# ooshyun/Speech-Enhancement-Pytorch

Measured on AMD Instinct MI355X. Metric: audio-sec/sec training, DCCRN 16kHz 2s bs32, higher is better.
Workload: dtype bf16; 1 GPU; DCCRN (kernel_num 16-32-64-128-256-256, complex LSTM 128, mask E) train step, 16 kHz 2-s clips, SI-SNR, Adam 3e-4, clip 5; per_gpu_batch=32, global_batch=32, samples_per_clip=32000, parallelism=dp1, launch=eager, inputs=resident in HBM

## Files before the change

### include/sehip.h

```cpp
#ifndef SEHIP_H
#define SEHIP_H
#include <stdint.h>

#ifdef __cplusplus
extern "C" {
#endif

const char* sehip_last_error(void);
const char* sehip_last_kernel(void);
int sehip_version(void);
int sehip_check_device(int device);

void* sehip_event_create(void);
int sehip_event_destroy(void* event);
int sehip_stream_depend(void* to_stream, void* from_stream, void* event);
int sehip_event_record(void* event, void* stream);
int sehip_stream_wait_event(void* stream, void* event);
void* sehip_stream_create(int priority_class);
int sehip_stream_destroy(void* stream);

int sehip_stft_frames(int n_samples, int win_len, int hop);
int sehip_stft_fwd(const float* wav , const float* window , int B, int N, int win_len, int hop,
                   int fft_len, float* spec , void* enc_in_bf16 , void* stream);
int sehip_istft_fwd(const float* spec, const float* mask , const float* window,
                    const float* inv_coff , int B, int T, int win_len, int hop, int fft_len, int length,
                    int masking_mode , float* frames_ws , float* wav ,
                    void* stream);
int sehip_istft_bwd(const float* dwav, const float* wav, const float* spec, const float* mask, const float* window,
                    const float* inv_coff, int B, int T, int win_len, int hop, int fft_len, int length,
                    int masking_mode, void* dmask_bf16 , void* stream);

int sehip_stft_custom_frames(int n_samples, int n_fft, int hop, int center);
int sehip_stft_custom_fwd(const float* wav, int rows, int n_samples, int n_fft, int hop, int win_length, int center,
                          float* spec, void* stream);
int sehip_istft_custom_fwd(const float* spec, int rows, int n_frames, int n_fft, int hop, int win_length, int center,
                           int length, float* frames_ws, float* wav, void* stream);

int sehip_wav_row_stats(const float* raw, const long* row_off, int rows, float* stats, void* stream);
int sehip_wav_collate(const float* raw, const long* row_off, const int* out_row, const long* out_start, const int* out_valid,
                      const float* stats, int mode, float eps, int seg, int out_rows, float* out, void* stream);

int sehip_sisnr_fwd(const float* est, const float* ref, int rows, int n, float* rowstat, float* loss, void* stream);
int sehip_sisdr_metric(const float* reference, const float* estimation, int rows, int n, float* ratios, float* out, void* stream);
int sehip_sisnr_bwd(const float* est, const float* ref, const float* rowstat, const float* upstream ,
                    int rows, int n, float* dest, void* stream);

int sehip_sisnr_pit_fwd(const float* est, const float* ref, int B, int S, int C, int n, float* rowstat, float* pairloss,
                        int* perm, float* loss, void* stream);
int sehip_sisnr_pit_bwd(const float* est, const float* ref, const float* rowstat, const int* perm, const float* upstream ,
                        int B, int S, int C, int n, float* dest, void* stream);

int sehip_psa_loss_fwd(const float* enh, const float* tgt, const float* mix, long ncomplex, double* acc, float* loss, void* stream);
int sehip_psa_loss_bwd(const float* enh, const float* tgt, const float* mix, long ncomplex, const float* upstream, float* denh, void* stream);
int sehip_pointwise_loss_fwd(const float* x, const float* y, long n, int mode, double* acc_scratch, float* loss, void* stream);
int sehip_pointwise_loss_bwd(const float* x, const float* y, long n, int mode, const float* upstream, float* dx, void* stream);

int sehip_grad_sumsq(const float* grads, long n, double* sumsq_out, void* stream);
int sehip_opt_step(float* params, float* grads, float* m, float* v, long n, const double* sumsq, float max_norm,
                   float lr, float beta1, float beta2, float eps, int step, const int* step_dev ,
                   float weight_decay, int mode, float grad_scale, void* stream);
// ... 297 lines not shown
```

### speech-enhancement-pytorch_amd/sehip/_lib.py

```python
import ctypes as C
import os

import torch

_HERE = os.path.dirname(os.path.abspath(__file__))
LIB_PATH = os.environ.get("SEHIP_LIB") or os.path.join(_HERE, "libsehip.so")


class SehipError(RuntimeError):
    pass


_lib = None

P = C.c_void_p
I = C.c_int
L = C.c_long
F = C.c_float
U = C.c_uint

_PROTOS = {
    "sehip_version": [],
    "sehip_check_device": [I],
    "sehip_set_deterministic": [I],
# ... 12 lines not shown
    "sehip_comm_unique_id": [P],
    "sehip_comm_init": [P, I, I, P],
    "sehip_allreduce_f32": [P, P, L, P],
    "sehip_allreduce_i32_max": [P, P, L, P],
    "sehip_comm_info": [P, P, P, P],
    "sehip_comm_destroy": [P],
    "sehip_wav_row_stats": [P, P, I, P, P],
    "sehip_wav_collate": [P, P, P, P, P, P, I, F, I, I, P, P],
    "sehip_sisnr_fwd": [P, P, I, I, P, P, P],
    "sehip_sisdr_metric": [P, P, I, I, P, P, P],
    "sehip_sisnr_bwd": [P, P, P, P, I, I, P, P],
    "sehip_sisnr_pit_fwd": [P, P, I, I, I, I, P, P, P, P, P],
    "sehip_sisnr_pit_bwd": [P, P, P, P, P, I, I, I, I, P, P],
    "sehip_psa_loss_fwd": [P, P, P, L, P, P, P],
    "sehip_psa_loss_bwd": [P, P, P, L, P, P, P],
    "sehip_pointwise_loss_fwd": [P, P, L, I, P, P, P],
    "sehip_pointwise_loss_bwd": [P, P, L, I, P, P, P],
    "sehip_grad_sumsq": [P, L, P, P],
    "sehip_opt_step": [P, P, P, P, L, P, F, F, F, F, F, I, P, F, I, F, P],
    "sehip_opt_step_g": [P, P, P, P, L, P, F, F, F, F, F, I, P, F, I, F, P, P],
    "sehip_opt_step_m": [P, P, P, P, L, P, F, F, F, F, F, I, P, F, I, F, P, P, I, P, P, P, P],
    "sehip_opt_begin_g": [P, I, P, P, I, P, P],
    "sehip_counter_add": [P, I, P],
    "sehip_zero_regions": [P, L, P, L, P, L, P, L, P],
    "sehip_gemm_takes_gln_stats": [P],
    "sehip_init": [],
    "sehip_grad_metric": [P, P, I, L, P, P, P, P],
    "sehip_opt_begin": [P, I, P, P, I, P],
    "sehip_grad_sumsq_acc": [P, L, P, P],
    "sehip_grad_metric_acc": [P, P, I, L, P, P, P, P],
    "sehip_cbn_scratch_floats": [L, I],
    "sehip_stft_fwd": [P, P, I, I, I, I, I, P, P, P],
    "sehip_istft_fwd": [P, P, P, P, I, I, I, I, I, I, I, P, P, P],
    "sehip_istft_bwd": [P, P, P, P, P, P, I, I, I, I, I, I, I, P, P],
    "sehip_gemm": [P, P],
    "sehip_gemm_pair": [P, P, P],
    "sehip_wgrad": [P, P],
    "sehip_wgrad_pair": [P, P, P],
    "sehip_bnr_rows": [P, P],
    "sehip_cbn_bwd_finalize_n": [P, I, P, P, P, P, L, I, P, P, P, P, P, P, P, P],
    "sehip_wgrad_group_bytes": [I],
    "sehip_wgrad_group_prepare": [P, I, P, P],
    "sehip_wgrad_group": [P, I, I, P],
    "sehip_wgrad_dense_group_bytes": [I],
    "sehip_wgrad_dense_group_prepare": [P, I, P, L, P],
    "sehip_wgrad_dense_group": [P, I, P, P, P],
    "sehip_gemm_desc_size": [],
    "sehip_conv_small_takes": [P, P],
    "sehip_pack_bf16": [P, P, L, P, P],
    "sehip_pack_f32": [P, P, L, P, P],
    "sehip_pack_head": [P, P, L, P, P, L, P, P, L, P],
    "sehip_unpack_grad": [P, P, L, P, P],
    "sehip_unpack_grad_sums": [P, P, L, P, P, I, P, P, P, P, P],
    "sehip_unpack_grad_sums_perm": [P, P, P, L, P, P, I, P, P, P, P, P],
    "sehip_unpack_grad1": [P, P, L, P, P],
    "sehip_unpack_grad1_sums": [P, P, L, P, P, I, P, P, P, P, P],
    "sehip_unpack_grad_list_sums": [P, P, P, L, P, P, I, P, P, P],
    "sehip_unpack_grad_list": [P, P, P, L, P, P],
    "sehip_pack_bf16_runs": [P, P, P, L, P, P],
    "sehip_pack_bf16_runs_to": [P, P, P, P, L, P, P],
    "sehip_cbn_stats": [P, L, I, P, P],
    "sehip_cbn_finalize": [P, P, P, P, P, P, P, P, P, P, P, P, L, I, F, F, I, P, P],
    "sehip_cbn_finalize_n": [P, I, P, P, P, P, P, P, P, P, P, P, P, L, I, F, F, I, P, P],
    "sehip_cbn_apply": [P, P, P, L, I, P, P],
    "sehip_cbn_finalize_apply_n": [P, P, I, P, P, P, P, P, P, P, P, P, P, P, L, I, F, F, I, P, P, P, P],
    "sehip_cbn_bwd_reduce": [P, P, P, P, P, L, I, I, I, I, P, P],
# ... 155 lines not shown
```

### speech-enhancement-pytorch_amd/sehip/csrc/stft.hip

```cpp
#include "common.h"

#include "fft512.h"
#include "mask.h"

__global__ __launch_bounds__(256) void stft_fwd_kernel(const float* __restrict__ wav, const float* __restrict__ window,
                                                       int B, int N, int T, int win, int hop,
                                                       float2* __restrict__ spec, unsigned* __restrict__ enc_in) {
    const int lane = threadIdx.x & 63;
    const int frame = blockIdx.x * 4 + (threadIdx.x >> 6);
    if (frame >= B * T) return;
    const int b = frame / T, t = frame - b * T;
    FftTw tw;
    fft_twiddles<-1>(tw, lane);
    float re[8], im[8];
    const int pad = win - hop;
    const float* x = wav + (size_t)b * N;
#pragma unroll
    for (int r = 0; r < 8; ++r) {
        const int n = lane + 64 * r;
        const int s = t * hop + n - pad;
        float v = 0.f;
        if (n < win && s >= 0 && s < N) v = x[s] * window[n];
        re[r] = v; im[r] = 0.f;
    }
    fft512_wave<-1>(re, im, tw, lane);
    __shared__ float2 srow[4][264 + 33];
    __shared__ unsigned senc[4][256];
    const int w = threadIdx.x >> 6;
    const int k0 = 8 * brev6(lane);
    constexpr int brev3[8] = {0, 4, 2, 6, 1, 5, 3, 7};
    if (k0 <= 256) {
#pragma unroll
        for (int j = 0; j < 8; ++j) {
            const int k = k0 + brev3[j];
            if (k <= 256) {
                srow[w][k + (k >> 3)] = make_float2(re[j], im[j]);
                if (k >= 1) senc[w][k - 1] = pack_bf2(re[j], im[j]);
            }
        }
    }
    __builtin_amdgcn_fence(__ATOMIC_RELEASE, "wavefront");
    __builtin_amdgcn_wave_barrier();
    __builtin_amdgcn_fence(__ATOMIC_ACQUIRE, "wavefront");
    float2* so = spec + (size_t)frame * NBIN;
    unsigned* eo = enc_in + (size_t)frame * 256;
#pragma unroll
    for (int j = 0; j < 4; ++j) {
        const int k = lane + 64 * j;
        so[k] = srow[w][k + (k >> 3)];
    }
    if (lane == 0) so[256] = srow[w][256 + 32];
    *reinterpret_cast<uint4*>(eo + 4 * lane) = *reinterpret_cast<const uint4*>(&senc[w][4 * lane]);
}

__global__ __launch_bounds__(256) void istft_frames_kernel(const float2* __restrict__ spec, const float2* __restrict__ mask,
                                                           const float* __restrict__ window, int nframes, int win, int mode,
                                                           float* __restrict__ frames) {
    const int lane = threadIdx.x & 63;
    const int frame = blockIdx.x * 4 + (threadIdx.x >> 6);
    if (frame >= nframes) return;
    FftTw tw;
    fft_twiddles<1>(tw, lane);
    float re[8], im[8];
    const float2* sp = spec + (size_t)frame * NBIN;
    const float2* mk = mask + (size_t)frame * 256;
#pragma unroll
    for (int r = 0; r < 8; ++r) {
        const int k = lane + 64 * r;
        float er = 0.f, ei = 0.f;
        if (k >= 1 && k <= 256) {
            const float2 z = sp[k];
            const float2 m = mk[k - 1];
            apply_mask(mode, z.x, z.y, m.x, m.y, er, ei);
        }
        re[r] = er; im[r] = ei;
    }
    fft512_wave<1>(re, im, tw, lane);
    const int n0 = 8 * brev6(lane);
    constexpr int brev3[8] = {0, 4, 2, 6, 1, 5, 3, 7};
    float u[8];
    float s1 = 0.f, s2 = 0.f;
#pragma unroll
    for (int j = 0; j < 8; ++j) {
        const int n = n0 + brev3[j];
        u[brev3[j]] = re[j];
        if (n < win) { s1 += re[j]; s2 += (n & 1) ? -re[j] : re[j]; }
    }
    s1 = wave_sum(s1);
    s2 = wave_sum(s2);
    const float c = 1.0f / (float)(FFT_N + win);
    float* fo = frames + (size_t)frame * win;
    if (n0 + 8 <= win && (win & 3) == 0) {
        float o[8];
#pragma unroll
        for (int q = 0; q < 8; ++q) {
            const int n = n0 + q;
            const float corr = c * (s1 + ((n & 1) ? -s2 : s2));
            o[q] = window[n] * (1.0f / 256.0f) * (u[q] - corr);
        }
        *reinterpret_cast<float4*>(fo + n0) = make_float4(o[0], o[1], o[2], o[3]);
        *reinterpret_cast<float4*>(fo + n0 + 4) = make_float4(o[4], o[5], o[6], o[7]);
        return;
    }
#pragma unroll
    for (int q = 0; q < 8; ++q) {
        const int n = n0 + q;
        if (n < win) {
            const float corr = c * (s1 + ((n & 1) ? -s2 : s2));
            fo[n] = window[n] * (1.0f / 256.0f) * (u[q] - corr);
        }
    }
}

__global__ __launch_bounds__(256) void istft_ola_kernel(const float* __restrict__ frames, const float* __restrict__ inv_coff,
                                                        int T, int win, int hop, int length, float* __restrict__ wav) {
    const int b = blockIdx.y;
    const int pad = win - hop;
    for (int i = blockIdx.x * 256 + threadIdx.x; i < length; i += gridDim.x * 256) {
        const int s = i + pad;
        int t_hi = s / hop;
        int t_lo = (s - win + hop) / hop;
        if (s - win + 1 <= 0) t_lo = 0;
        if (t_hi > T - 1) t_hi = T - 1;
        float acc = 0.f;
        for (int t = t_lo; t <= t_hi; ++t) acc += frames[((size_t)b * T + t) * win + (s - t * hop)];
        acc *= inv_coff[i];
        wav[(size_t)b * length + i] = fminf(1.f, fmaxf(-1.f, acc));
    }
}

__global__ __launch_bounds__(256) void istft_bwd_kernel(const float* __restrict__ dwav, const float* __restrict__ wav,
                                                        const float* __restrict__ inv_coff, const float* __restrict__ window,
                                                        const float2* __restrict__ spec, const float2* __restrict__ mask,
                                                        int B, int T, int win, int hop, int length, int mode,
                                                        unsigned* __restrict__ dmask_bf16) {
    const int lane = threadIdx.x & 63;
    const int frame = blockIdx.x * 4 + (threadIdx.x >> 6);
    if (frame >= B * T) return;
    const int b = frame / T, t = frame - b * T;
    FftTw tw;
    fft_twiddles<-1>(tw, lane);
    const int pad = win - hop;
    float re[8], im[8];
    float s1 = 0.f, s2 = 0.f;
#pragma unroll
    for (int r = 0; r < 8; ++r) {
        const int n = lane + 64 * r;
        const int i = t * hop + n - pad;
        float v = 0.f;
        if (n < win && i >= 0 && i < length) {
            const size_t o = (size_t)b * length + i;
            const float y = wav[o];
            if (y > -1.f && y < 1.f) v = dwav[o] * inv_coff[i] * window[n] * (1.0f / 256.0f);
        }
        re[r] = v; im[r] = 0.f;
        s1 += v; s2 += (n & 1) ? -v : v;
    }
    s1 = wave_sum(s1);
    s2 = wave_sum(s2);
    const float c = 1.0f / (float)(FFT_N + win);
#pragma unroll
    for (int r = 0; r < 8; ++r) {
        const int n = lane + 64 * r;
        if (n < win) re[r] -= c * (s1 + ((n & 1) ? -s2 : s2));
    }
    const float2* sp = spec + (size_t)frame * NBIN;
    const float2* mk = mask + (size_t)frame * 256;
    float2 spv[4], mkv[4];
#pragma unroll
    for (int j = 0; j < 4; ++j) { spv[j] = sp[1 + lane + 64 * j]; mkv[j] = mk[lane + 64 * j]; }
    fft512_wave<-1>(re, im, tw, lane);
    __shared__ float2 ssp[4][256 + 32], smk[4][256 + 32];
    __shared__ unsigned sdm[4][256];
    const int w = threadIdx.x >> 6;
#pragma unroll
    for (int j = 0; j < 4; ++j) {
        const int i = lane + 64 * j;
        ssp[w][i + (i >> 3)] = spv[j];
        smk[w][i + (i >> 3)] = mkv[j];
    }
    __builtin_amdgcn_fence(__ATOMIC_RELEASE, "wavefront");
    __builtin_amdgcn_wave_barrier();
    __builtin_amdgcn_fence(__ATOMIC_ACQUIRE, "wavefront");
    const int k0 = 8 * brev6(lane);
    constexpr int brev3[8] = {0, 4, 2, 6, 1, 5, 3, 7};
    if (k0 <= 256) {
#pragma unroll
        for (int j = 0; j < 8; ++j) {
            const int k = k0 + brev3[j];
            if (k < 1 || k > 256) continue;
            const float dr = re[j], di = im[j];
            const int i = k - 1;
            const float2 z = ssp[w][i + (i >> 3)];
            const float2 m = smk[w][i + (i >> 3)];
            float gmr, gmi;
            mask_grad(mode, z.x, z.y, m.x, m.y, dr, di, gmr, gmi);
            sdm[w][i] = pack_bf2(gmr, gmi);
        }
    }
    __builtin_amdgcn_fence(__ATOMIC_RELEASE, "wavefront");
    __builtin_amdgcn_wave_barrier();
    __builtin_amdgcn_fence(__ATOMIC_ACQUIRE, "wavefront");
    unsigned* dm = dmask_bf16 + (size_t)frame * 256;
    *reinterpret_cast<uint4*>(dm + 4 * lane) = *reinterpret_cast<const uint4*>(&sdm[w][4 * lane]);
}

static int check_stft_cfg(const char* who, int win, int hop, int fft) {
    SEHIP_REQUIRE(fft == FFT_N, "%s: only fft_len 512 is built (got %d)", who, fft);
    SEHIP_REQUIRE(win > 0 && win <= FFT_N && (win % 2) == 0, "%s: win_len must be even and <= 512 (got %d)", who, win);
    SEHIP_REQUIRE(hop > 0 && hop <= win, "%s: bad hop %d", who, hop);
    return 0;
}

extern "C" int sehip_stft_frames(int n_samples, int win, int hop) { return (n_samples + 2 * (win - hop) - win) / hop + 1; }

extern "C" int sehip_stft_fwd(const float* wav, const float* window, int B, int N, int win, int hop, int fft, float* spec,
                              void* enc_in_bf16, void* stream) {
    if (int e = check_stft_cfg("stft_fwd", win, hop, fft)) return e;
    SEHIP_REQUIRE(B > 0 && N > 0, "stft_fwd: empty input");
    const int T = sehip_stft_frames(N, win, hop);
    SEHIP_REQUIRE(T > 0, "stft_fwd: input shorter than one frame");
    stft_fwd_kernel<<<cdiv((long)B * T, 4), 256, 0, (hipStream_t)stream>>>(wav, window, B, N, T, win, hop, (float2*)spec,
                                                                           (unsigned*)enc_in_bf16);
    SEHIP_CHECK_LAUNCH("stft_fwd");
    return 0;
}

extern "C" int sehip_istft_fwd(const float* spec, const float* mask, const float* window, const float* inv_coff, int B,
                               int T, int win, int hop, int fft, int length, int mode, float* frames_ws, float* wav,
                               void* stream) {
    if (int e = check_stft_cfg("istft_fwd", win, hop, fft)) return e;
    SEHIP_REQUIRE(B > 0 && T > 0 && length > 0, "istft_fwd: empty input");
    SEHIP_REQUIRE(mode >= 0 && mode <= 2, "istft_fwd: masking mode must be 0(E) 1(C) 2(R)");
    SEHIP_REQUIRE(length <= (T - 1) * hop + win - (win - hop), "istft_fwd: length %d exceeds the synthesised signal", length);
    hipStream_t st = (hipStream_t)stream;
    istft_frames_kernel<<<cdiv((long)B * T, 4), 256, 0, st>>>((const float2*)spec, (const float2*)mask, window, B * T, win,
                                                             mode, frames_ws);
    dim3 grid(cdiv(length, 256 * 4), B);
    istft_ola_kernel<<<grid, 256, 0, st>>>(frames_ws, inv_coff, T, win, hop, length, wav);
    SEHIP_CHECK_LAUNCH("istft_fwd");
    return 0;
}

extern "C" int sehip_istft_bwd(const float* dwav, const float* wav, const float* spec, const float* mask,
                               const float* window, const float* inv_coff, int B, int T, int win, int hop, int fft,
                               int length, int mode, void* dmask_bf16, void* stream) {
    if (int e = check_stft_cfg("istft_bwd", win, hop, fft)) return e;
    SEHIP_REQUIRE(B > 0 && T > 0 && length > 0, "istft_bwd: empty input");
    SEHIP_REQUIRE(mode >= 0 && mode <= 2, "istft_bwd: masking mode must be 0(E) 1(C) 2(R)");
    istft_bwd_kernel<<<cdiv((long)B * T, 4), 256, 0, (hipStream_t)stream>>>(dwav, wav, inv_coff, window, (const float2*)spec,
                                                                            (const float2*)mask, B, T, win, hop, length, mode,
                                                                            (unsigned*)dmask_bf16);
    SEHIP_CHECK_LAUNCH("istft_bwd");
    return 0;
}
```

### speech-enhancement-pytorch_amd/sehip/model/dccrn.py

```python
import os
import numpy as np
import torch
from torch import nn

from .. import plan, ops
from .._lib import SehipError
from .flat import FlatModule, _Node

_STATIC_CACHE = {}


def _static_for(cfg, deterministic=False):
    switches = tuple(os.environ.get(k) for k in ("SEHIP_NO_FUSE_STATS", "SEHIP_NO_FUSE_STATS64", "SEHIP_NO_FUSE_STATS32", "SEHIP_DEC_SPLIT"))
    key = (tuple(cfg.kernel_num), cfg.rnn_layers, cfg.rnn_units, cfg.win_len, cfg.win_inc, cfg.fft_len, cfg.length, cfg.masking_mode, str(cfg.win_type), bool(cfg.use_cbn), bool(cfg.use_clstm), switches,
           bool(deterministic))
    if key not in _STATIC_CACHE:
        _STATIC_CACHE[key] = plan.DCCRNStatic(cfg, deterministic=deterministic)
    return _STATIC_CACHE[key]


class _DCCRNFunction(torch.autograd.Function):
    @staticmethod
    def forward(ctx, model, wav, anchor):
        ctx.model = model
        ctx.ws = model._run_forward(wav)
        ctx.generation = ctx.ws.generation
        return ctx.ws.wav.view(wav.shape[0], 1, -1).clone()

    @staticmethod
    def backward(ctx, grad_out):
        if ctx.generation != ctx.ws.generation or ctx.ws.closed:
            raise SehipError("DCCRN.backward: the workspace of this forward was overwritten by a later forward of the same "
                             "shape (or evicted); run backward before the next forward of that shape")
        from .._lib import stream_scope
        with stream_scope():
            ctx.model._run_backward(ctx.ws, grad_out)
        return None, None, None


class DCCRN(FlatModule):
    def __init__(self, rnn_layers=2, rnn_units=128, win_len=400, win_inc=100, fft_len=512, length=16384, win_type="hann",
                 masking_mode="E", use_clstm=True, use_cbn=True, kernel_size=5, kernel_num=[16, 32, 64, 128, 256, 256],
                 *args, **kwargs):
        super().__init__()
        self.cfg = cfg = plan.DCCRNConfig(rnn_layers=rnn_layers, rnn_units=rnn_units, win_len=win_len, win_inc=win_inc,
                                          fft_len=fft_len, length=length, win_type=win_type, masking_mode=masking_mode,
                                          use_clstm=use_clstm, use_cbn=use_cbn, kernel_size=kernel_size,
                                          kernel_num=list(kernel_num))
        self.win_len, self.win_inc, self.fft_len, self.rnn_units = win_len, win_inc, fft_len, rnn_units
        self.masking_mode, self.kernel_num = masking_mode, cfg.kernel_num
        self.static = _static_for(cfg)
        self._tables = None
        self._ws_cap = max(1, int(os.environ.get("SEHIP_WS_CACHE", "4")))
        self.grad_range_hook = None

        an, sy, win = _stft_bases(win_len, fft_len, win_type)
        self.stft = _Node()
        self.stft.register_buffer("weight", torch.from_numpy(an[:, None, :]))
        self.istft = _Node()
        self.istft.register_buffer("weight", torch.from_numpy(sy[:, None, :]))
# ... 36 lines not shown

    def set_deterministic(self, on=True):
        on = bool(on)
        if on == self.static.deterministic:
            return self
        self.static = _static_for(self.cfg, deterministic=on)
        self._tables = None
        for ws in list(self._ws.values()):
            ws.close()
        self._ws.clear()
        self._last_ws = None
        return self

    step_guard_early = True

    def step_guard(self):
        ws = getattr(self, "_last_ws", None)
        return ws.l2_sync[0:1] if ws is not None and hasattr(ws, "l2_sync") else None

    def check_health(self):
        from ..distrib import global_flag
        ws = getattr(self, "_last_ws", None)
        if ws is None:
            return global_flag(False, self._flat.device if self._flat is not None else None)
        lost = bool(ws.check_lstm_handoffs(recover=True, global_flag=global_flag))
        self._note_graph_epoch(ws)
        return lost

    def _run_forward(self, wav):
        ws = self.workspace(wav.shape[0], wav.shape[-1])
        self._last_ws = ws
        ws.generation += 1
        x = wav.reshape(wav.shape[0], wav.shape[-1]).contiguous().float()
        ws.forward(x, self._flat, self._bflat, self._nbt, training=self.training)
        return ws

    def _run_backward(self, ws, grad_out):
        if not self.training:
            raise SehipError("DCCRN.backward in eval mode (running-statistics BatchNorm) is not built")
        g = grad_out.reshape(ws.B, ws.length).contiguous().float()
        accumulating = self._grads_live and self._params[0][1].grad is not None
        hook = self.grad_range_hook if not accumulating else None
        tail = self._tail_sink if (hook is None and not accumulating) else None
        self._backward_into_flat(lambda dst: ws.backward(g, self._flat, dst, range_ready=hook, tail=tail))
        if tail is not None:
            self._tail_done = self._tail_counted = self._tail_dirty = True
        else:
            self._tail_done = False

    def forward(self, inputs, lens=None):
        if inputs.dim() == 2:
            inputs = inputs.unsqueeze(1)
        if not inputs.is_cuda:
            raise SehipError("DCCRN.forward got a CPU tensor: the HIP path needs a gfx950 GPU (no CPU fallback)")
        if torch.is_grad_enabled() and self.training:
            if self._anchor is None or self._anchor.device != inputs.device:
                self._anchor = torch.zeros(1, device=inputs.device, requires_grad=True)
            return _DCCRNFunction.apply(self, inputs, self._anchor)
        ws = self._run_forward(inputs)
        return ws.wav.view(inputs.shape[0], 1, -1).clone()

    def get_params(self, weight_decay=0.0):
        weights, biases = [], []
        for name, p in self.named_parameters():
            (biases if "bias" in name else weights).append(p)
        return [{"params": weights, "weight_decay": weight_decay}, {"params": biases, "weight_decay": 0.0}]


def _stft_bases(win_len, fft_len, win_type="hann"):
    n = np.arange(win_len, dtype=np.float64)[None, :]
    k = np.arange(fft_len // 2 + 1, dtype=np.float64)[:, None]
    ang = 2.0 * np.pi * k * n / fft_len
    basis = np.concatenate([np.cos(ang), -np.sin(ang)], axis=0)
    win = ops.window_of(win_type, win_len).astype(np.float64)
    return ((basis * win).astype(np.float32), (np.linalg.pinv(basis).T * win).astype(np.float32), win.astype(np.float32))
```

### speech-enhancement-pytorch_amd/sehip/plan.py

```python
import ctypes as C
import os
import math

import numpy as np
import torch

from . import _lib
from ._lib import call, ptr, stream, SehipError
from . import ops

BF16 = torch.bfloat16


class CSrc(C.Structure):
    _fields_ = [("ptr", C.c_void_p), ("T", C.c_int32), ("tlo", C.c_int32), ("thi", C.c_int32), ("F", C.c_int32),
                ("C", C.c_int32), ("pad_", C.c_int32)]


class CDst(C.Structure):
    _fields_ = [("ptr", C.c_void_p), ("T", C.c_int32), ("F", C.c_int32), ("C", C.c_int32), ("toff", C.c_int32),
                ("fmul", C.c_int32), ("fadd", C.c_int32), ("is_f32", C.c_int32), ("tmul", C.c_int32)]


class CGemmDesc(C.Structure):
# ... 794 lines not shown
                add(f"dz{i}", T, f, c)
        c5, h = kn[6], cfg.hid
        add("dz5l", T, 4, c5); add("P", T, 4, c5); add("dP", T, 4, c5)
        L = cfg.rnn_layers
        if not cfg.use_clstm:
            for layer in (1, 2):
                add(f"pre{layer}", T, 1, 4 * h, dtype=torch.float32)
                add(f"dpre{layer}", T, 1, 4 * h)
                add(f"h{layer}", T, 1, h, lead=1)
                add(f"gates{layer}", T, 1, 4 * h, lead=1, batch=Bp)
                add(f"c{layer}", T, 1, h, dtype=torch.float32, lead=1, batch=Bp)
            add("dxo", T, 1, h); add("dx2", T, 1, h)
        for layer in range(1, L + 1 if cfg.use_clstm else 0):
            for tag in "ri":
                add(f"pre{layer}_{tag}", T, 1, 8 * h, dtype=torch.float32)
                add(f"dpre{layer}_{tag}", T, 1, 8 * h)
            add(f"h{layer}", T, 1, h, lead=4)
            add(f"gates{layer}", T, 1, 4 * h, lead=4, batch=Bp)
            add(f"c{layer}", T, 1, h, dtype=torch.float32, lead=4, batch=Bp)
        for tag in ("ri" if cfg.use_clstm else ""):
            add(f"dxo_{tag}", T, 1, h)
            for layer in range(2, L + 1):
                add(f"dx{layer}_{tag}", T, 1, h)
        for j in range(5):
            idx = 6 - j
            f, c = (F0 >> idx) * 2, kn[idx - 1]
            add(f"yd{j}", T + 1, f, c, 1); add(f"zd{j}", T + 1, f, c, 1)
            add(f"dyd{j}", T + 1, f, c, 1); add(f"dzd{j}", T + 1, f, c, 1)
            if j in st.dec_split:
                add(f"pd{j}", T + 1, f, c, 1)
        add("mask", T, F0, 2, dtype=torch.float32)
        add("dmask", T, F0, 2)
        self.spec = torch.empty(B, T, 257, 2, dtype=torch.float32, device=device)
        self.frames = torch.empty(B, T, cfg.win_len, dtype=torch.float32, device=device)
        self.wav = torch.empty(B, self.length, dtype=torch.float32, device=device)
        self.inv_coff = torch.from_numpy(ops.inv_window_energy(cfg.win_len, cfg.win_inc, T, self.length, cfg.win_type)).to(device)
        self.gpack = torch.zeros(st.n_gpack, dtype=torch.float32, device=device)
        maxcr = max(cr for _, cr in st.bn)
        lib = _lib.lib()
        need = 16
        for pre, cr in st.bn:
            src = self.bufs[("y" if pre.startswith("encoder") else "yd") + pre.split(".")[1]]
            need = max(need, int(lib.sehip_cbn_scratch_floats(src.t.numel() // (2 * cr), cr)))
        self.bn_acc = torch.zeros(need, dtype=torch.float32, device=device)
        self.bn_coef = {pre: torch.zeros(cr, 16, dtype=torch.float32, device=device) for pre, cr in st.bn}
        offs, tot = {}, 0
        for pre, cr in st.bn:
            if pre in st.fused_stats or pre in st.small_stats:
                offs[pre] = tot
                tot += 8 * 5 * cr
        self.bn_stats_all = torch.zeros(max(tot, 1), dtype=torch.float32, device=device)
        self.fuse_finalize = not os.environ.get("SEHIP_NO_FUSE_FINALIZE")
        self.fuse_bwd_finalize = (self.fuse_finalize and not st.deterministic and bool(os.environ.get("SEHIP_FUSE_BWD_FINALIZE")))
        self.bn_reduce_fin = (self.fuse_finalize and not st.deterministic and not self.fuse_bwd_finalize
                              and bool(os.environ.get("SEHIP_BN_REDUCE_FIN")))
        self.bn_ticket = torch.zeros(len(st.bn) + 1, dtype=torch.int32, device=device)
        self._bn_index = {pre: i for i, (pre, _) in enumerate(st.bn)}
        self.fuse_bwd_all = bool(os.environ.get("SEHIP_FUSE_BWD_ALL"))
        self.bn_brep = {pre: torch.zeros(2, BWD_REPLICAS * (6 * cr + 1), dtype=torch.float32, device=device) for pre, cr in st.bn}
        self._brep_turn = {pre: 0 for pre, _ in st.bn}
        self.bn_stats = {pre: self.bn_stats_all[o:o + 8 * 5 * cr] for (pre, cr) in st.bn if pre in offs for o in [offs[pre]]}
        self.bn_bcoef = torch.zeros(maxcr, 16, dtype=torch.float32, device=device)
        self.bn_eps = 1e-5 if cfg.use_cbn else -1e-5
        self.bn_zero = torch.zeros(maxcr, dtype=torch.float32, device=device)
        self.bn_dummy = torch.zeros(maxcr, dtype=torch.float32, device=device)
        self._bn_cr = {pre: cr for pre, cr in st.bn}
        self.mode = {"E": 0, "C": 1, "R": 2}[cfg.masking_mode]
# ... 503 lines not shown
            wp = tb.wpack.data_ptr()
            call("sehip_lstm2_bwd", b["dxo_r"].ptr, b["dxo_i"].ptr, wp + 2 * st.whhT_off[1], wp + 2 * st.whhT_off[2],
                 wp + 2 * st.wihT2_off, b["gates1"].ptr, b["c1"].ptr, b["gates2"].ptr, b["c2"].ptr, B, T, h, b["dpre1_r"].ptr,
                 b["dpre1_i"].ptr, b["dpre2_r"].ptr, b["dpre2_i"].ptr, ptr(self.l2_gran_b), ptr(self.l2_sync),
                 getattr(self, "_l2_cur_epoch", 1), main)
            self._chain_dirty = True
            self.wgrad_group(self._lstm_wgrad_names((2, 1)))
            self.gemm_pair("dx1_r", "dx1_i")
            return
        nl = self.st.cfg.rnn_layers
        if self.lstm_stream is None or nl != 2 or torch.cuda.is_current_stream_capturing():
            for layer in range(nl, 0, -1):
                self._lstm_bwd_call(layer, 0, T, main)
                self.wgrad_group(self._lstm_wgrad_names((layer,)))
                self.gemm_pair(f"dx{layer}_r", f"dx{layer}_i")
            return
        s2, s3 = self.lstm_stream.cuda_stream, self.lstm_gemm_stream.cuda_stream
        for (t0, t1) in reversed(self.lstm_chunks):
            self._lstm_bwd_call(2, t0, t1, main)
            call("sehip_stream_depend", s3, main, self._event())
            call("sehip_gemm_pair", C.byref(self._chunk_desc("dx2_r", t0, t1)), C.byref(self._chunk_desc("dx2_i", t0, t1)), s3)
            call("sehip_stream_depend", s2, s3, self._event())
            self._lstm_bwd_call(1, t0, t1, s2)
        call("sehip_stream_depend", main, s2, self._event())
        self._chain_dirty = True
        self.wgrad_group(self._lstm_wgrad_names((2, 1)))
        self.gemm_pair("dx1_r", "dx1_i")

    def pack_weights(self, params):
        st, tb = self.st, self.tb
        call("sehip_pack_bf16", ptr(params), ptr(tb.wtab), st.n_wpack, ptr(tb.wpack), stream())
        call("sehip_pack_f32", ptr(params), ptr(tb.btab), st.n_bpack, ptr(tb.bpack), stream())

    def forward(self, wav_in, params, buffers, nbt, training=True):
        st, cfg, b, tb = self.st, self.st.cfg, self.bufs, self.tb
        B, T, h = self.B, self.T, cfg.hid
        zero = self.bn_stats_all if (self.st.fused_stats or self.fused_small) else None
        head = self.side.cuda_stream if (self.side is not None and PARALLEL_HEAD) else stream()
        if head != stream():
            call("sehip_stream_depend", head, stream(), self._event())
        call("sehip_pack_head", ptr(params), ptr(tb.wtab), st.n_wpack, ptr(tb.wpack), ptr(tb.btab), st.n_bpack, ptr(tb.bpack),
             ptr(zero) if zero is not None else None, zero.numel() if zero is not None else 0, head)
        if head != stream() and training:
            with torch.cuda.stream(self.side):
                self.gpack.zero_()
            self._gpack_clean = True
        call("sehip_stft_fwd", ptr(wav_in), ptr(tb.window), B, self.N, cfg.win_len, cfg.win_inc, cfg.fft_len,
             ptr(self.spec), b["enc_in"].ptr, stream())
        if head != stream():
            call("sehip_stream_depend", stream(), head, self._event())
        for i in range(6):
            self.gemm(f"enc{i}.fwd")
            self.bn_forward(f"encoder.{i}.", cfg.kernel_num[i + 1] // 2, b[f"y{i}"], b[f"z{i}"], params, buffers, nbt, training)
        split = st.dec_split if self.side is not None else []
        if split:
            sd = self.side.cuda_stream
            call("sehip_stream_depend", sd, stream(), self._event())
            if not self._fs_events:
                for _ in range(6):
                    e = _lib.lib().sehip_event_create()
                    if not e:
                        raise SehipError("sehip_event_create: " + _lib.lib().sehip_last_error().decode())
                    self._fs_events.append(e)
            for j in split:
                call("sehip_gemm_pair", C.byref(self.desc[f"dec{j}.fs0"]), C.byref(self.desc[f"dec{j}.fs1"]), sd)
                call("sehip_event_record", self._fs_events[j], sd)
        self._lstm_forward(B, T, h)
        if cfg.use_clstm:
            self.gemm_pair("proj_r", "proj_i")
        else:
            self.gemm("proj")
        for j in range(6):
            if j in split:
                call("sehip_stream_wait_event", stream(), self._fs_events[j])
                self.gemm_pair(f"dec{j}.fm0", f"dec{j}.fm1")
            else:
                self.gemm_pair(f"dec{j}.fwd0", f"dec{j}.fwd1")
            if j < 5:
                self.bn_forward(f"decoder.{j}.", cfg.kernel_num[5 - j] // 2, b[f"yd{j}"], b[f"zd{j}"], params, buffers, nbt,
                                training)
        call("sehip_istft_fwd", ptr(self.spec), b["mask"].ptr, ptr(tb.window), ptr(self.inv_coff), B, T, cfg.win_len,
             cfg.win_inc, cfg.fft_len, self.length, self.mode, ptr(self.frames), ptr(self.wav), stream())
        return self.wav

    def backward(self, dwav, params, grads, range_ready=None, tail=None):
        st, cfg, b, tb = self.st, self.st.cfg, self.bufs, self.tb
        B, T, h = self.B, self.T, cfg.hid
        if not getattr(self, "_gpack_clean", False):
            self.gpack.zero_()
        self._gpack_clean = False
        self._chain_dirty = True
        call("sehip_istft_bwd", ptr(dwav), ptr(self.wav), ptr(self.spec), b["mask"].ptr, ptr(tb.window), ptr(self.inv_coff),
             B, T, cfg.win_len, cfg.win_inc, cfg.fft_len, self.length, self.mode, b["dmask"].ptr, stream())
        for j in range(5, -1, -1):
            if j < 5:
                self.bn_backward(f"decoder.{j}.", cfg.kernel_num[5 - j] // 2, b[f"dzd{j}"], None, b[f"yd{j}"], b[f"dyd{j}"],
                                 params, 1)
            self.wgrad_pair(f"dec{j}.fwd0", f"dec{j}.fwd1")
            if j >= 1 and f"decoder.{j - 1}." in self.bnr_rows:
                self.desc[f"dec{j}.dg"].bnr_slope = params.data_ptr() + 4 * st.layout.param_off[f"decoder.{j - 1}.2.weight"][0]
            self.gemm(f"dec{j}.dg")
        if cfg.use_clstm:
            for tag in "ri":
                self.wgrad(f"proj_{tag}")
            self.gemm_pair("dproj_r", "dproj_i")
        else:
            self.wgrad("proj")
            self.gemm("dproj")
        self._lstm_backward(B, T, h)
        n_params = st.layout.n_params
        lo = st.layout.param_off["decoder.0.0.real_conv.weight"][0] if range_ready is not None else 0
        if range_ready is not None:
            L = st.layout
            if not getattr(st, "_dp_layout_checked", False):
                for nm in L.param_names:
# ... 42 lines not shown
```

Baseline: 19960 audio-s/s.

## Fuse iSTFT synthesis and overlap-add into one kernel with paired real IFFTs

Replaces the separate per-frame inverse FFT kernel plus overlap-add kernel with one kernel. Each block synthesises a run of frames (with halo) into LDS and overlap-adds them directly into the waveform, also writing the output copy so the later clone is dropped. Two real frames are packed into one complex 512-point IFFT per wave, halving FFT work, and the frames workspace round-trip through HBM is removed. The halo frames are recomputed across neighbouring blocks, and the istft backward is refactored into helpers with no intended speed change.

Result: no change. 20030 audio-s/s (median of 6 runs) (+0.4%).

```diff
diff --git a/include/sehip.h b/include/sehip.h
--- a/include/sehip.h
+++ b/include/sehip.h
@@ -26,6 +26,10 @@
                     const float* inv_coff , int B, int T, int win_len, int hop, int fft_len, int length,
                     int masking_mode , float* frames_ws , float* wav ,
                     void* stream);
+int sehip_istft_synth_run(int win_len, int hop);
+int sehip_istft_synth(const float* spec, const float* mask, const float* window, const float* inv_coff, int B, int T, int win_len,
+                      int hop, int fft_len, int length, int masking_mode, float* wav ,
+                      float* wav_copy , void* stream);
 int sehip_istft_bwd(const float* dwav, const float* wav, const float* spec, const float* mask, const float* window,
                     const float* inv_coff, int B, int T, int win_len, int hop, int fft_len, int length,
                     int masking_mode, void* dmask_bf16 , void* stream);
diff --git a/speech-enhancement-pytorch_amd/sehip/_lib.py b/speech-enhancement-pytorch_amd/sehip/_lib.py
--- a/speech-enhancement-pytorch_amd/sehip/_lib.py
+++ b/speech-enhancement-pytorch_amd/sehip/_lib.py
@@ -68,6 +68,8 @@
     "sehip_cbn_scratch_floats": [L, I],
     "sehip_stft_fwd": [P, P, I, I, I, I, I, P, P, P],
     "sehip_istft_fwd": [P, P, P, P, I, I, I, I, I, I, I, P, P, P],
+    "sehip_istft_synth_run": [I, I],
+    "sehip_istft_synth": [P, P, P, P, I, I, I, I, I, I, I, P, P, P],
     "sehip_istft_bwd": [P, P, P, P, P, P, I, I, I, I, I, I, I, P, P],
     "sehip_gemm": [P, P],
     "sehip_gemm_pair": [P, P, P],
diff --git a/speech-enhancement-pytorch_amd/sehip/csrc/stft.hip b/speech-enhancement-pytorch_amd/sehip/csrc/stft.hip
--- a/speech-enhancement-pytorch_amd/sehip/csrc/stft.hip
+++ b/speech-enhancement-pytorch_amd/sehip/csrc/stft.hip
@@ -53,62 +53,157 @@
     *reinterpret_cast<uint4*>(eo + 4 * lane) = *reinterpret_cast<const uint4*>(&senc[w][4 * lane]);
 }
 
-__global__ __launch_bounds__(256) void istft_frames_kernel(const float2* __restrict__ spec, const float2* __restrict__ mask,
-                                                           const float* __restrict__ window, int nframes, int win, int mode,
-                                                           float* __restrict__ frames) {
-    const int lane = threadIdx.x & 63;
-    const int frame = blockIdx.x * 4 + (threadIdx.x >> 6);
-    if (frame >= nframes) return;
-    FftTw tw;
-    fft_twiddles<1>(tw, lane);
-    float re[8], im[8];
+#define SY_WAVES 8
+#define SY_NF 15
+#define SY_MAX_HALO 3
+
+__device__ __forceinline__ void fetch_bins(const float2* __restrict__ spec, const float2* __restrict__ mask, long frame, bool valid,
+                                           int lane, float2 (&z)[4], float2 (&m)[4]) {
     const float2* sp = spec + (size_t)frame * NBIN;
     const float2* mk = mask + (size_t)frame * 256;
 #pragma unroll
-    for (int r = 0; r < 8; ++r) {
-        const int k = lane + 64 * r;
-        float er = 0.f, ei = 0.f;
-        if (k >= 1 && k <= 256) {
-            const float2 z = sp[k];
-            const float2 m = mk[k - 1];
-            apply_mask(mode, z.x, z.y, m.x, m.y, er, ei);
-        }
-        re[r] = er; im[r] = ei;
-    }
-    fft512_wave<1>(re, im, tw, lane);
-    const int n0 = 8 * brev6(lane);
+    for (int r = 0; r < 4; ++r) {
+        int k = lane + 64 * r;
+        if (k == 0) k = 256;
+        z[r] = valid ? sp[k] : make_float2(0.f, 0.f);
+        m[r] = valid ? mk[k - 1] : make_float2(0.f, 0.f);
+    }
+}
+
+__device__ __forceinline__ bool masked_bins(const float2 (&z)[4], const float2 (&m)[4], bool valid, int mode, float (&er)[4],
+                                            float (&ei)[4]) {
+    bool nz = false;
+#pragma unroll
+    for (int r = 0; r < 4; ++r) {
+        er[r] = 0.f; ei[r] = 0.f;
+        if (valid) apply_mask(mode, z[r].x, z[r].y, m[r].x, m[r].y, er[r], ei[r]);
+        nz = nz || er[r] != 0.f || ei[r] != 0.f;
+    }
+    return __any(nz) != 0;
+}
+
+__device__ __forceinline__ void synth_emit(const float (&x)[8], bool nz, const float (&wv)[8], int n0, int win, float (&o)[8]) {
     constexpr int brev3[8] = {0, 4, 2, 6, 1, 5, 3, 7};
     float u[8];
     float s1 = 0.f, s2 = 0.f;
 #pragma unroll
     for (int j = 0; j < 8; ++j) {
         const int n = n0 + brev3[j];
-        u[brev3[j]] = re[j];
-        if (n < win) { s1 += re[j]; s2 += (n & 1) ? -re[j] : re[j]; }
+        u[brev3[j]] = x[j];
+        if (n < win) { s1 += x[j]; s2 += (n & 1) ? -x[j] : x[j]; }
     }
     s1 = wave_sum(s1);
     s2 = wave_sum(s2);
     const float c = 1.0f / (float)(FFT_N + win);
-    float* fo = frames + (size_t)frame * win;
-    if (n0 + 8 <= win && (win & 3) == 0) {
-        float o[8];
-#pragma unroll
-        for (int q = 0; q < 8; ++q) {
-            const int n = n0 + q;
-            const float corr = c * (s1 + ((n & 1) ? -s2 : s2));
-            o[q] = window[n] * (1.0f / 256.0f) * (u[q] - corr);
-        }
-        *reinterpret_cast<float4*>(fo + n0) = make_float4(o[0], o[1], o[2], o[3]);
-        *reinterpret_cast<float4*>(fo + n0 + 4) = make_float4(o[4], o[5], o[6], o[7]);
-        return;
-    }
 #pragma unroll
     for (int q = 0; q < 8; ++q) {
         const int n = n0 + q;
-        if (n < win) {
-            const float corr = c * (s1 + ((n & 1) ? -s2 : s2));
-            fo[n] = window[n] * (1.0f / 256.0f) * (u[q] - corr);
+        const float corr = c * (s1 + ((n & 1) ? -s2 : s2));
+        const float v = wv[q] * (1.0f / 256.0f) * (u[q] - corr);
+        o[q] = (nz && n < win) ? v : 0.f;
+    }
+}
+
+__device__ __forceinline__ void synth_pair(const float2* __restrict__ spec, const float2* __restrict__ mask,
+                                           const float* __restrict__ window, long nframes, int win, int mode, long pair, int lane,
+                                           float (&oa)[8], float (&ob)[8]) {
+    const long fa = 2 * pair, fb = fa + 1;
+    float2 z1[4], m1[4], z2[4], m2[4];
+    fetch_bins(spec, mask, fa, true, lane, z1, m1);
+    fetch_bins(spec, mask, fb, fb < nframes, lane, z2, m2);
+    float e1r[4], e1i[4], e2r[4], e2i[4];
+    const bool nza = masked_bins(z1, m1, true, mode, e1r, e1i);
+    const bool nzb = masked_bins(z2, m2, fb < nframes, mode, e2r, e2i);
+    float cr[4], ci[4];
+#pragma unroll
+    for (int q = 0; q < 4; ++q) { cr[q] = e1r[q] + e2i[q]; ci[q] = e2r[q] - e1i[q]; }
+    if (lane == 0) { cr[0] = 2.f * e1r[0]; ci[0] = 2.f * e2r[0]; }
+    const int src = (64 - lane) & 63;
+    float re[8], im[8];
+#pragma unroll
+    for (int r = 0; r < 4; ++r) {
+        re[r] = 0.5f * (e1r[r] - e2i[r]);
+        im[r] = 0.5f * (e1i[r] + e2r[r]);
+        const float mr = lane == 0 ? cr[(4 - r) & 3] : cr[3 - r], mi = lane == 0 ? ci[(4 - r) & 3] : ci[3 - r];
+        re[4 + r] = 0.5f * __shfl(mr, src, 64);
+        im[4 + r] = 0.5f * __shfl(mi, src, 64);
+    }
+    if (lane == 0) { re[0] = 0.f; im[0] = 0.f; }
+    FftTw tw;
+    fft_twiddles<1>(tw, lane);
+    fft512_wave<1>(re, im, tw, lane);
+    const int n0 = 8 * brev6(lane);
+    float wv[8];
+#pragma unroll
+    for (int q = 0; q < 8; ++q) wv[q] = n0 + q < win ? window[n0 + q] : 0.f;
+    synth_emit(re, nza, wv, n0, win, oa);
+    synth_emit(im, nzb, wv, n0, win, ob);
+}
+
+__device__ __forceinline__ void store_frame(float* __restrict__ row, const float (&o)[8], int n0, int win) {
+    if (n0 + 8 <= win && (win & 3) == 0) {
+        *reinterpret_cast<float4*>(row + n0) = make_float4(o[0], o[1], o[2], o[3]);
+        *reinterpret_cast<float4*>(row + n0 + 4) = make_float4(o[4], o[5], o[6], o[7]);
+        return;
+    }
+#pragma unroll
+    for (int q = 0; q < 8; ++q)
+        if (n0 + q < win) row[n0 + q] = o[q];
+}
+
+__global__ __launch_bounds__(64 * SY_WAVES) void istft_synth_kernel(const float2* __restrict__ spec, const float2* __restrict__ mask,
+                                                                    const float* __restrict__ window,
+                                                                    const float* __restrict__ inv_coff, int B, int T, int win, int hop,
+                                                                    int length, int mode, int run, float* __restrict__ frames,
+                                                                    float* __restrict__ wav, float* __restrict__ wav_copy) {
+    extern __shared__ float sfr[];
+    const int lane = threadIdx.x & 63, w = threadIdx.x >> 6;
+    const long nframes = (long)B * T;
+    const int n0 = 8 * brev6(lane);
+    const int b = blockIdx.y, t0 = blockIdx.x * run, pad = win - hop;
+    int s_lo = 0, s_hi = 0;
+    long g_lo, g_hi;
+    if (frames != nullptr) {
+        g_lo = (long)blockIdx.x * (2 * SY_WAVES);
+        g_hi = min(g_lo + 2 * SY_WAVES, nframes) - 1;
+    } else {
+        s_lo = max(t0 * hop, pad);
+        s_hi = min(t0 + run >= T ? (T - 1) * hop + win : (t0 + run) * hop, length + pad);
+        if (s_lo >= s_hi) return;
+        const int t_first = s_lo - win + 1 <= 0 ? 0 : (s_lo - win + hop) / hop;
+        const int t_last = min((s_hi - 1) / hop, T - 1);
+        g_lo = (long)b * T + t_first;
+        g_hi = (long)b * T + t_last;
+    }
+    const long p_lo = g_lo >> 1, p_hi = g_hi >> 1;
+    const long pair = p_lo + w;
+    if (pair <= p_hi) {
+        float oa[8], ob[8];
+        synth_pair(spec, mask, window, nframes, win, mode, pair, lane, oa, ob);
+        const long fa = 2 * pair;
+        if (frames != nullptr) {
+            store_frame(frames + (size_t)fa * win, oa, n0, win);
+            if (fa + 1 <= g_hi) store_frame(frames + (size_t)(fa + 1) * win, ob, n0, win);
+        } else {
+            if (fa >= g_lo) store_frame(sfr + (size_t)(fa - 2 * p_lo) * win, oa, n0, win);
+            if (fa + 1 <= g_hi) store_frame(sfr + (size_t)(fa + 1 - 2 * p_lo) * win, ob, n0, win);
         }
+    }
+    if (frames != nullptr) return;
+    __syncthreads();
+    const long f0 = (long)b * T - 2 * p_lo;
+    for (int s = s_lo + threadIdx.x; s < s_hi; s += 64 * SY_WAVES) {
+        const int i = s - pad;
+        int t_hi = s / hop;
+        int t_lo = (s - win + hop) / hop;
+        if (s - win + 1 <= 0) t_lo = 0;
+        if (t_hi > T - 1) t_hi = T - 1;
+        float acc = 0.f;
+        for (int t = t_lo; t <= t_hi; ++t) acc += sfr[(f0 + t) * win + (s - t * hop)];
+        acc *= inv_coff[i];
+        const float v = fminf(1.f, fmaxf(-1.f, acc));
+        wav[(size_t)b * length + i] = v;
+        if (wav_copy != nullptr) wav_copy[(size_t)b * length + i] = v;
     }
 }
 
@@ -129,80 +224,103 @@
     }
 }
 
+__device__ __forceinline__ void istft_bwd_input(const float* __restrict__ dwav, const float* __restrict__ wav,
+                                                const float* __restrict__ inv_coff, const float* __restrict__ window, long frame,
+                                                int T, int win, int hop, int length, int lane, float (&x)[8]) {
+    const int b = (int)(frame / T), t = (int)(frame - (long)b * T);
+    const int pad = win - hop;
+    float y[8], d[8], ic[8], wn[8];
+    bool ok[8];
+#pragma unroll
+    for (int r = 0; r < 8; ++r) {
+        const int n = lane + 64 * r;
+        const int i = t * hop + n - pad;
+        ok[r] = n < win && i >= 0 && i < length;
+        const size_t o = ok[r] ? (size_t)b * length + i : 0;
+        y[r] = wav[o];
+        d[r] = dwav[o];
+        ic[r] = inv_coff[ok[r] ? i : 0];
+        wn[r] = window[ok[r] ? n : 0];
+    }
+    float s1 = 0.f, s2 = 0.f;
+#pragma unroll
+    for (int r = 0; r < 8; ++r) {
+        const int n = lane + 64 * r;
+        float v = 0.f;
+        if (ok[r] && y[r] > -1.f && y[r] < 1.f) v = d[r] * ic[r] * wn[r] * (1.0f / 256.0f);
+        x[r] = v;
+        s1 += v; s2 += (n & 1) ? -v : v;
+    }
+    s1 = wave_sum(s1);
+    s2 = wave_sum(s2);
+    const float c = 1.0f / (float)(FFT_N + win);
+#pragma unroll
+    for (int r = 0; r < 8; ++r) {
+        const int n = lane + 64 * r;
+        if (n < win) x[r] -= c * (s1 + ((n & 1) ? -s2 : s2));
+    }
+}
+
+__device__ __forceinline__ void istft_bwd_emit(float2* __restrict__ ssp, float2* __restrict__ smk, unsigned* __restrict__ sdm,
+                                               const float2 (&spv)[4], const float2 (&mkv)[4], const float (&dr_)[8],
+                                               const float (&di_)[8], int mode, int lane, unsigned* __restrict__ dm) {
+#pragma unroll
+    for (int j = 0; j < 4; ++j) {
+        const int i = lane + 64 * j;
+        ssp[i + (i >> 3)] = spv[j];
+        smk[i + (i >> 3)] = mkv[j];
+    }
+    __builtin_amdgcn_fence(__ATOMIC_RELEASE, "wavefront");
+    __builtin_amdgcn_wave_barrier();
+    __builtin_amdgcn_fence(__ATOMIC_ACQUIRE, "wavefront");
+    const int k0 = 8 * brev6(lane);
+    constexpr int brev3[8] = {0, 4, 2, 6, 1, 5, 3, 7};
+    if (k0 <= 256) {
+#pragma unroll
+        for (int j = 0; j < 8; ++j) {
+            const int k = k0 + brev3[j];
+            if (k < 1 || k > 256) continue;
+            const float dr = dr_[j], di = di_[j];
+            const int i = k - 1;
+            const float2 z = ssp[i + (i >> 3)];
+            const float2 m = smk[i + (i >> 3)];
+            float gmr, gmi;
+            mask_grad(mode, z.x, z.y, m.x, m.y, dr, di, gmr, gmi);
+            sdm[i] = pack_bf2(gmr, gmi);
+        }
+    }
+    __builtin_amdgcn_fence(__ATOMIC_RELEASE, "wavefront");
+    __builtin_amdgcn_wave_barrier();
+    __builtin_amdgcn_fence(__ATOMIC_ACQUIRE, "wavefront");
+    *reinterpret_cast<uint4*>(dm + 4 * lane) = *reinterpret_cast<const uint4*>(&sdm[4 * lane]);
+}
+
 __global__ __launch_bounds__(256) void istft_bwd_kernel(const float* __restrict__ dwav, const float* __restrict__ wav,
                                                         const float* __restrict__ inv_coff, const float* __restrict__ window,
                                                         const float2* __restrict__ spec, const float2* __restrict__ mask,
                                                         int B, int T, int win, int hop, int length, int mode,
                                                         unsigned* __restrict__ dmask_bf16) {
     const int lane = threadIdx.x & 63;
-    const int frame = blockIdx.x * 4 + (threadIdx.x >> 6);
-    if (frame >= B * T) return;
-    const int b = frame / T, t = frame - b * T;
+    const long nframes = (long)B * T;
+    const long fa = (long)blockIdx.x * 4 + (threadIdx.x >> 6);
+    if (fa >= nframes) return;
     FftTw tw;
     fft_twiddles<-1>(tw, lane);
-    const int pad = win - hop;
     float re[8], im[8];
-    float s1 = 0.f, s2 = 0.f;
-#pragma unroll
-    for (int r = 0; r < 8; ++r) {
-        const int n = lane + 64 * r;
-        const int i = t * hop + n - pad;
-        float v = 0.f;
-        if (n < win && i >= 0 && i < length) {
-            const size_t o = (size_t)b * length + i;
-            const float y = wav[o];
-            if (y > -1.f && y < 1.f) v = dwav[o] * inv_coff[i] * window[n] * (1.0f / 256.0f);
-        }
-        re[r] = v; im[r] = 0.f;
-        s1 += v; s2 += (n & 1) ? -v : v;
-    }
-    s1 = wave_sum(s1);
-    s2 = wave_sum(s2);
-    const float c = 1.0f / (float)(FFT_N + win);
-#pragma unroll
-    for (int r = 0; r < 8; ++r) {
-        const int n = lane + 64 * r;
-        if (n < win) re[r] -= c * (s1 + ((n & 1) ? -s2 : s2));
-    }
-    const float2* sp = spec + (size_t)frame * NBIN;
-    const float2* mk = mask + (size_t)frame * 256;
-    float2 spv[4], mkv[4];
-#pragma unroll
-    for (int j = 0; j < 4; ++j) { spv[j] = sp[1 + lane + 64 * j]; mkv[j] = mk[lane + 64 * j]; }
+    istft_bwd_input(dwav, wav, inv_coff, window, fa, T, win, hop, length, lane, re);
+#pragma unroll
+    for (int j = 0; j < 8; ++j) im[j] = 0.f;
+    float2 spa[4], mka[4];
+#pragma unroll
+    for (int j = 0; j < 4; ++j) {
+        spa[j] = spec[(size_t)fa * NBIN + 1 + lane + 64 * j];
+        mka[j] = mask[(size_t)fa * 256 + lane + 64 * j];
+    }
     fft512_wave<-1>(re, im, tw, lane);
     __shared__ float2 ssp[4][256 + 32], smk[4][256 + 32];
     __shared__ unsigned sdm[4][256];
     const int w = threadIdx.x >> 6;
-#pragma unroll
-    for (int j = 0; j < 4; ++j) {
-        const int i = lane + 64 * j;
-        ssp[w][i + (i >> 3)] = spv[j];
-        smk[w][i + (i >> 3)] = mkv[j];
-    }
-    __builtin_amdgcn_fence(__ATOMIC_RELEASE, "wavefront");
-    __builtin_amdgcn_wave_barrier();
-    __builtin_amdgcn_fence(__ATOMIC_ACQUIRE, "wavefront");
-    const int k0 = 8 * brev6(lane);
-    constexpr int brev3[8] = {0, 4, 2, 6, 1, 5, 3, 7};
-    if (k0 <= 256) {
-#pragma unroll
-        for (int j = 0; j < 8; ++j) {
-            const int k = k0 + brev3[j];
-            if (k < 1 || k > 256) continue;
-            const float dr = re[j], di = im[j];
-            const int i = k - 1;
-            const float2 z = ssp[w][i + (i >> 3)];
-            const float2 m = smk[w][i + (i >> 3)];
-            float gmr, gmi;
-            mask_grad(mode, z.x, z.y, m.x, m.y, dr, di, gmr, gmi);
-            sdm[w][i] = pack_bf2(gmr, gmi);
-        }
-    }
-    __builtin_amdgcn_fence(__ATOMIC_RELEASE, "wavefront");
-    __builtin_amdgcn_wave_barrier();
-    __builtin_amdgcn_fence(__ATOMIC_ACQUIRE, "wavefront");
-    unsigned* dm = dmask_bf16 + (size_t)frame * 256;
-    *reinterpret_cast<uint4*>(dm + 4 * lane) = *reinterpret_cast<const uint4*>(&sdm[w][4 * lane]);
+    istft_bwd_emit(ssp[w], smk[w], sdm[w], spa, mka, re, im, mode, lane, dmask_bf16 + (size_t)fa * 256);
 }
 
 static int check_stft_cfg(const char* who, int win, int hop, int fft) {
@@ -233,12 +351,38 @@
     SEHIP_REQUIRE(B > 0 && T > 0 && length > 0, "istft_fwd: empty input");
     SEHIP_REQUIRE(mode >= 0 && mode <= 2, "istft_fwd: masking mode must be 0(E) 1(C) 2(R)");
     SEHIP_REQUIRE(length <= (T - 1) * hop + win - (win - hop), "istft_fwd: length %d exceeds the synthesised signal", length);
+    SEHIP_REQUIRE(frames_ws != nullptr, "istft_fwd: no frames workspace");
     hipStream_t st = (hipStream_t)stream;
-    istft_frames_kernel<<<cdiv((long)B * T, 4), 256, 0, st>>>((const float2*)spec, (const float2*)mask, window, B * T, win,
-                                                             mode, frames_ws);
+    istft_synth_kernel<<<cdiv(cdiv((long)B * T, 2), SY_WAVES), 64 * SY_WAVES, 0, st>>>((const float2*)spec, (const float2*)mask, window,
+                                                                                      inv_coff, B, T, win, hop, length, mode, 0,
+                                                                                      frames_ws, nullptr, nullptr);
     dim3 grid(cdiv(length, 256 * 4), B);
     istft_ola_kernel<<<grid, 256, 0, st>>>(frames_ws, inv_coff, T, win, hop, length, wav);
     SEHIP_CHECK_LAUNCH("istft_fwd");
+    return 0;
+}
+
+extern "C" int sehip_istft_synth_run(int win, int hop) {
+    if (win <= 0 || hop <= 0 || hop > win) return 0;
+    const int halo = (win - 1) / hop;
+    return halo <= SY_MAX_HALO ? SY_NF - halo : 0;
+}
+
+extern "C" int sehip_istft_synth(const float* spec, const float* mask, const float* window, const float* inv_coff, int B, int T,
+                                 int win, int hop, int fft, int length, int mode, float* wav, float* wav_copy, void* stream) {
+    if (int e = check_stft_cfg("istft_synth", win, hop, fft)) return e;
+    SEHIP_REQUIRE(B > 0 && T > 0 && length > 0, "istft_synth: empty input");
+    SEHIP_REQUIRE(mode >= 0 && mode <= 2, "istft_synth: masking mode must be 0(E) 1(C) 2(R)");
+    SEHIP_REQUIRE(length <= (T - 1) * hop + win - (win - hop), "istft_synth: length %d exceeds the synthesised signal", length);
+    const int run = sehip_istft_synth_run(win, hop);
+    SEHIP_REQUIRE(run > 0, "istft_synth: win_len %d / hop %d needs more than %d halo frames per run: call sehip_istft_fwd", win, hop,
+                  SY_MAX_HALO);
+    SEHIP_REQUIRE(wav != nullptr, "istft_synth: no output");
+    dim3 grid(cdiv(T, run), B);
+    const size_t lds = (size_t)(SY_NF + 1) * win * sizeof(float);
+    istft_synth_kernel<<<grid, 64 * SY_WAVES, lds, (hipStream_t)stream>>>((const float2*)spec, (const float2*)mask, window, inv_coff,
+                                                                          B, T, win, hop, length, mode, run, nullptr, wav, wav_copy);
+    SEHIP_CHECK_LAUNCH("istft_synth");
     return 0;
 }
 
diff --git a/speech-enhancement-pytorch_amd/sehip/model/dccrn.py b/speech-enhancement-pytorch_amd/sehip/model/dccrn.py
--- a/speech-enhancement-pytorch_amd/sehip/model/dccrn.py
+++ b/speech-enhancement-pytorch_amd/sehip/model/dccrn.py
@@ -23,9 +23,9 @@
     @staticmethod
     def forward(ctx, model, wav, anchor):
         ctx.model = model
-        ctx.ws = model._run_forward(wav)
+        ctx.ws, out = model._run_forward(wav)
         ctx.generation = ctx.ws.generation
-        return ctx.ws.wav.view(wav.shape[0], 1, -1).clone()
+        return out
 
     @staticmethod
     def backward(ctx, grad_out):
@@ -128,8 +128,9 @@
         self._last_ws = ws
         ws.generation += 1
         x = wav.reshape(wav.shape[0], wav.shape[-1]).contiguous().float()
-        ws.forward(x, self._flat, self._bflat, self._nbt, training=self.training)
-        return ws
+        out = torch.empty(wav.shape[0], 1, ws.length, dtype=torch.float32, device=wav.device)
+        ws.forward(x, self._flat, self._bflat, self._nbt, training=self.training, out=out)
+        return ws, out
 
     def _run_backward(self, ws, grad_out):
         if not self.training:
@@ -153,8 +154,7 @@
             if self._anchor is None or self._anchor.device != inputs.device:
                 self._anchor = torch.zeros(1, device=inputs.device, requires_grad=True)
             return _DCCRNFunction.apply(self, inputs, self._anchor)
-        ws = self._run_forward(inputs)
-        return ws.wav.view(inputs.shape[0], 1, -1).clone()
+        return self._run_forward(inputs)[1]
 
     def get_params(self, weight_decay=0.0):
         weights, biases = [], []
diff --git a/speech-enhancement-pytorch_amd/sehip/plan.py b/speech-enhancement-pytorch_amd/sehip/plan.py
--- a/speech-enhancement-pytorch_amd/sehip/plan.py
+++ b/speech-enhancement-pytorch_amd/sehip/plan.py
@@ -850,7 +850,8 @@
         add("mask", T, F0, 2, dtype=torch.float32)
         add("dmask", T, F0, 2)
         self.spec = torch.empty(B, T, 257, 2, dtype=torch.float32, device=device)
-        self.frames = torch.empty(B, T, cfg.win_len, dtype=torch.float32, device=device)
+        self.frames = None if _lib.lib().sehip_istft_synth_run(cfg.win_len, cfg.win_inc) > 0 else \
+            torch.empty(B, T, cfg.win_len, dtype=torch.float32, device=device)
         self.wav = torch.empty(B, self.length, dtype=torch.float32, device=device)
         self.inv_coff = torch.from_numpy(ops.inv_window_energy(cfg.win_len, cfg.win_inc, T, self.length, cfg.win_type)).to(device)
         self.gpack = torch.zeros(st.n_gpack, dtype=torch.float32, device=device)
@@ -1420,7 +1421,7 @@
         call("sehip_pack_bf16", ptr(params), ptr(tb.wtab), st.n_wpack, ptr(tb.wpack), stream())
         call("sehip_pack_f32", ptr(params), ptr(tb.btab), st.n_bpack, ptr(tb.bpack), stream())
 
-    def forward(self, wav_in, params, buffers, nbt, training=True):
+    def forward(self, wav_in, params, buffers, nbt, training=True, out=None):
         st, cfg, b, tb = self.st, self.st.cfg, self.bufs, self.tb
         B, T, h = self.B, self.T, cfg.hid
         zero = self.bn_stats_all if (self.st.fused_stats or self.fused_small) else None
@@ -1467,8 +1468,14 @@
             if j < 5:
                 self.bn_forward(f"decoder.{j}.", cfg.kernel_num[5 - j] // 2, b[f"yd{j}"], b[f"zd{j}"], params, buffers, nbt,
                                 training)
-        call("sehip_istft_fwd", ptr(self.spec), b["mask"].ptr, ptr(tb.window), ptr(self.inv_coff), B, T, cfg.win_len,
-             cfg.win_inc, cfg.fft_len, self.length, self.mode, ptr(self.frames), ptr(self.wav), stream())
+        if self.frames is None:
+            call("sehip_istft_synth", ptr(self.spec), b["mask"].ptr, ptr(tb.window), ptr(self.inv_coff), B, T, cfg.win_len,
+                 cfg.win_inc, cfg.fft_len, self.length, self.mode, ptr(self.wav), ptr(out), stream())
+        else:
+            call("sehip_istft_fwd", ptr(self.spec), b["mask"].ptr, ptr(tb.window), ptr(self.inv_coff), B, T, cfg.win_len,
+                 cfg.win_inc, cfg.fft_len, self.length, self.mode, ptr(self.frames), ptr(self.wav), stream())
+            if out is not None:
+                out.view(self.wav.shape).copy_(self.wav)
         return self.wav
 
     def backward(self, dwav, params, grads, range_ready=None, tail=None):
```
